# ZpokenWeb3/zk-light-client-implementation

Hardware: AMD Instinct MI355X
Metric: Block_i BFT-finality proofs/sec (100 validators) (higher is better)
Workload: dtype u64

## Files before the change

__graft_entry__.py:

```python
import os
import subprocess
import sys

ROOT = os.path.dirname(os.path.abspath(__file__))
if ROOT not in sys.path:
    sys.path.insert(0, ROOT)


def build() -> None:
    import concurrent.futures
    import importlib
    b = importlib.import_module("zk-light-client-implementation_amd.build")
    pool = concurrent.futures.ThreadPoolExecutor(max_workers=1)
    devsim = pool.submit(b.build_devsim, True)
    b.build(verbose=True)
    mk = os.path.join(ROOT, "oracle", "c", "Makefile")
    if os.path.exists(mk):
        subprocess.check_call(["make", "-s", "-C", os.path.dirname(mk)])
    import zklc_amd
    zklc_amd.load()
    lib_dir = os.path.join(ROOT, "zk-light-client-implementation_amd", "lib")
    subprocess.check_call(["gcc", "-O2", "-Wall", "-Wextra", "-std=c11", "-D_POSIX_C_SOURCE=200809L", "-I", os.path.join(ROOT, "include"),
                           os.path.join(ROOT, "tests", "c_abi", "prove_from_file.c"), "-o", os.path.join(ROOT, "tests", "c_abi", "prove_from_file"),
                           "-L", lib_dir, "-lzklc_mi355", "-Wl,-rpath,$ORIGIN/../../zk-light-client-implementation_amd/lib"])
    b.build_poseidon_gate_dev(True)
    b.build_fri_coeff_dev(True)
    devsim.result()
    pool.shutdown()


def smoke() -> None:
    import json
    import numpy as np
    import zklc_amd
    from oracle import ed25519_ref as ref

    with zklc_amd.Context(0) as ctx:
        j = json.load(open(os.path.join(ROOT, "tests", "golden", "ed25519_near_c1_small.json")))
        msg = bytes.fromhex(j["msg"])
        pks = b"".join(bytes.fromhex(e["validator_tail"])[1:33] for e in j["entries"])
        sigs = b"".join(bytes.fromhex(e["approval"])[2:] for e in j["entries"])
        ok = ctx.ed25519_verify_batch(pks, sigs, msg)
        exp = [int(ref.verify(pks[32 * i:32 * i + 32], sigs[64 * i:64 * i + 64], msg)) for i in range(len(ok))]
        assert ok.tolist() == exp == [1, 1, 1], (ok.tolist(), exp)
        m2 = b"zklc smoke"
        pk2, sg2, exp2 = [], [], []
        for i in range(64):
            sd = ref.synthetic_seed(11, i)
            _, _, pk = ref.keypair(sd)
            s = bytearray(ref.sign(sd, m2))
            if i % 5 == 4:
                s[i % 64] ^= 0x10
            pk2.append(pk)
            sg2.append(bytes(s))
            exp2.append(int(ref.verify(pk, bytes(s), m2)))
        ok2 = ctx.ed25519_verify_batch(b"".join(pk2), b"".join(sg2), m2)
        assert ok2.tolist() == exp2, "GPU Ed25519 batch differs from the oracle"
        assert sum(exp2) == 64 - 12
        from zklc_amd.plonky2 import CircuitBuilder, serialization as S, HASH_GL
        from oracle import plonky2_prover as OP, plonky2_verifier as V
        b = CircuitBuilder()
        x = b.add_virtual_public_input()
        y = b.add_virtual_target()
        z = b.mul(x, y)
        b.split_le(x, 10)
        lo, hi = b.mul_add_u32(x, y, b.constant(77))
        b.register_public_input(lo)
        b.connect(b.sub(b.add(z, b.constant(5)), z), b.constant(5))
        data = b.build()
        wires, pis = data.generate_witness({x: 1000, y: 4000000000})
        prover = data.prover(ctx, HASH_GL)
        raw = prover.prove_bytes(wires, pis)
        common = data.common_data()
        oproof, ovd = OP.prove(common, data.constants, data.sigmas, wires, pis, V.HasherGL)
        assert raw == S.proof_to_bytes(oproof, common, HASH_GL), "GPU plonky2 proof differs from the oracle prover"
        V.verify(json.loads(json.dumps(S.proof_from_bytes(raw, common, HASH_GL))), prover.verifier_data(), common)
        from zklc_amd.plonky2.recursion import RecursionProver
        rp = RecursionProver(ctx, HASH_GL)
        rc, rproof = rp.recursive_proof((common, prover.verifier_data(), raw), None, [7, 8])
        V.verify(json.loads(json.dumps(rproof)), rc.verifier_only, rc.common)
        assert rproof["public_inputs"] == [7, 8]
        bad = bytearray(raw)
        bad[800] ^= 1
        try:
            rp.recursive_proof((common, prover.verifier_data(), bytes(bad)), None, [7, 8])
            raise SystemExit("smoke: a tampered inner proof was accepted by the in-circuit verifier")
        except AssertionError:
            pass
        rp.close()
        prover.close()
    print("smoke OK: Ed25519 batch verify, a plonky2 proof and a recursive proof on cuda:0 match the oracle")


if __name__ == "__main__":
    build()
    if "--smoke" in sys.argv:
        smoke()
```

zk-light-client-implementation_amd/build.py:

```python
import concurrent.futures as cf
import glob
import os
import subprocess
import sys

HERE = os.path.dirname(os.path.abspath(__file__))
CSRC = os.path.join(HERE, "csrc")
BUILD = os.path.join(HERE, "build")
LIBDIR = os.path.join(HERE, "lib")
LIB = os.path.join(LIBDIR, "libzklc_mi355.so")
HIPCC = os.environ.get("HIPCC", "/opt/rocm/bin/hipcc")
FLAGS = ["--offload-arch=gfx950", "-O3", "-std=c++17", "-fPIC", "-fno-gpu-rdc", "-Wall", "-Wno-unused-function"]


def _newest(paths):
    return max((os.path.getmtime(p) for p in paths), default=0.0)


HOST_CXX = os.environ.get("CXX", "g++")
HOST_FLAGS = ["-O3", "-funroll-loops", "-std=c++17", "-fPIC", "-pthread", "-Wall", "-Wno-unused-function", "-Wno-unknown-pragmas"]


def _compile(src, obj, log):
    cmd = ([HIPCC] + FLAGS if src.endswith(".hip") else [HOST_CXX] + HOST_FLAGS) + ["-c", src, "-o", obj]
# ... 20 lines not shown
            jobs.append((s, o))
    if jobs:
        with cf.ThreadPoolExecutor(max_workers=min(len(jobs), os.cpu_count() or 4)) as ex:
            list(ex.map(lambda so: _compile(so[0], so[1], verbose), jobs))
    if jobs or not os.path.exists(LIB) or os.path.getmtime(LIB) < _newest(objs):
        cmd = [HIPCC, "--offload-arch=gfx950", "-shared", "-fPIC", "-pthread", "-o", LIB] + objs
        r = subprocess.run(cmd, capture_output=True, text=True)
        if r.returncode != 0:
            raise RuntimeError("link failed:\n%s\n%s" % (r.stdout, r.stderr))
        if verbose:
            print("[zklc build] linked", LIB, file=sys.stderr)
    return LIB


DEVSIM_DIR = os.path.join(HERE, "..", "tests", "devsim")
DEVSIM_SRC = os.path.join(DEVSIM_DIR, "devsim.hip")
DEVSIM_LIB = os.path.join(DEVSIM_DIR, "libdevsim.so")


def devsim_sources():
    return [DEVSIM_SRC, os.path.abspath(__file__)] + [p for ext in ("*.cuh", "*.h", "*.inc") for p in glob.glob(os.path.join(CSRC, ext))]


def devsim_is_current():
    return os.path.exists(DEVSIM_LIB) and os.path.getmtime(DEVSIM_LIB) >= _newest(devsim_sources())


def build_devsim(verbose=True, force=False):
    if force or not devsim_is_current():
        r = subprocess.run([HIPCC] + FLAGS + ["-shared", DEVSIM_SRC, "-o", DEVSIM_LIB], capture_output=True, text=True)
        if r.returncode != 0:
            raise RuntimeError("hipcc failed for %s:\n%s\n%s" % (DEVSIM_SRC, r.stdout, r.stderr))
        if verbose:
            print("[zklc build] built", DEVSIM_LIB, file=sys.stderr)
    return DEVSIM_LIB


PGD_DIR = os.path.join(HERE, "..", "tests", "poseidon_gate_dev")
PGD_SRC = os.path.join(PGD_DIR, "poseidon_gate_dev.hip")
PGD_LIB = os.path.join(PGD_DIR, "libposeidon_gate_dev.so")


def poseidon_gate_dev_is_current():
    deps = [PGD_SRC, os.path.abspath(__file__)] + [p for ext in ("*.cuh", "*.h", "*.inc") for p in glob.glob(os.path.join(CSRC, ext))]
    return os.path.exists(PGD_LIB) and os.path.getmtime(PGD_LIB) >= _newest(deps)


def build_poseidon_gate_dev(verbose=True, force=False):
    if force or not poseidon_gate_dev_is_current():
        r = subprocess.run([HIPCC] + FLAGS + ["-Wno-inline-asm", "-shared", PGD_SRC, "-o", PGD_LIB], capture_output=True, text=True)
        if r.returncode != 0:
            raise RuntimeError("hipcc failed for %s:\n%s\n%s" % (PGD_SRC, r.stdout, r.stderr))
        if verbose:
            print("[zklc build] built", PGD_LIB, file=sys.stderr)
    return PGD_LIB


FCD_DIR = os.path.join(HERE, "..", "tests", "fri_coeff_dev")
FCD_SRC = os.path.join(FCD_DIR, "fri_coeff_dev.hip")
FCD_CASES = os.path.join(FCD_DIR, "fri_coeff_dev_cases.cpp")
FCD_LIB = os.path.join(FCD_DIR, "libfri_coeff_dev.so")


def fri_coeff_dev_is_current():
    deps = [FCD_SRC, FCD_CASES, os.path.join(HERE, "..", "tests", "fri_coeff_host", "fri_coeff_cases.h"), os.path.abspath(__file__)]
    deps += [p for ext in ("*.cuh", "*.h", "*.inc") for p in glob.glob(os.path.join(CSRC, ext))]
    return os.path.exists(FCD_LIB) and os.path.getmtime(FCD_LIB) >= _newest(deps)


def build_fri_coeff_dev(verbose=True, force=False):
    if force or not fri_coeff_dev_is_current():
        obj, kobj = os.path.join(FCD_DIR, "fri_coeff_dev_cases.o"), os.path.join(FCD_DIR, "fri_coeff_dev.o")
        for cmd in ([HOST_CXX, "-O2", "-std=c++17", "-fPIC", "-Wall", "-Wno-unused-function", "-Wno-unknown-pragmas", "-c", FCD_CASES, "-o", obj],
                    [HIPCC] + FLAGS + ["-c", FCD_SRC, "-o", kobj],
                    [HIPCC, "--offload-arch=gfx950", "-shared", "-fPIC", "-o", FCD_LIB, kobj, obj]):
            r = subprocess.run(cmd, capture_output=True, text=True)
            if r.returncode != 0:
                raise RuntimeError("%s failed for %s:\n%s\n%s" % (cmd[0], FCD_DIR, r.stdout[-4000:], r.stderr[-4000:]))
        if verbose:
            print("[zklc build] built", FCD_LIB, file=sys.stderr)
    return FCD_LIB


if __name__ == "__main__":
    build(force="--force" in sys.argv)
    build_devsim(force="--force" in sys.argv)
    build_poseidon_gate_dev(force="--force" in sys.argv)
    build_fri_coeff_dev(force="--force" in sys.argv)
```

zk-light-client-implementation_amd/csrc/plonky2_prover.hip:

```cpp
#include <algorithm>
#include <chrono>
#include <stdio.h>
#include <stdlib.h>
#include <new>
#include <vector>
#include <string.h>
#include "plonky2_gates.cuh"
#include "plonky2_host.h"
#include "plonky2_perm_terms.cuh"
#include "plonky2_fri_combine.cuh"
#include "zklc_internal.h"

#define P2_THREADS 256

struct p2_challenges {
    u64 beta[P2_MAX_CH], gamma[P2_MAX_CH], alpha[P2_MAX_CH];
};

__global__ void p2_pow_table_kernel(u64 *out, u64 base, u64 n) {
    u64 i = (u64)blockIdx.x * blockDim.x + threadIdx.x;
    if (i < n) out[i] = gl_pow(base, i);
}

__global__ void p2_scale_by_powers_kernel(u64 *data, u64 base, u64 n) {
    u64 j = (u64)blockIdx.x * blockDim.x + threadIdx.x;
    if (j >= n) return;
    u64 *p = data + (size_t)blockIdx.y * n + j;
    *p = gl_mul(*p, gl_pow(base, j));
}

#define P2_SCALE_PER_LANE 8
__global__ void __launch_bounds__(256) p2_scale_by_powers_strided_kernel(u64 *data, u64 base, u64 step, u64 n) {
    const u64 j0 = (u64)blockIdx.x * (256 * P2_SCALE_PER_LANE) + threadIdx.x;
    if (j0 >= n) return;
    u64 *p = data + (size_t)blockIdx.y * n;
    u64 v[P2_SCALE_PER_LANE];
#pragma unroll
    for (int q = 0; q < P2_SCALE_PER_LANE; q++) v[q] = j0 + 256 * q < n ? p[j0 + 256 * q] : 0;
    u64 pw = gl_pow(base, j0);
#pragma unroll
    for (int q = 0; q < P2_SCALE_PER_LANE; q++) {
        if (j0 + 256 * q < n) p[j0 + 256 * q] = gl_mul(v[q], pw);
        if (q + 1 < P2_SCALE_PER_LANE) pw = gl_mul(pw, step);
    }
}

__global__ void p2_ext_powers_kernel(gl2 *out, gl2 z, u64 n) {
    u64 j = (u64)blockIdx.x * blockDim.x + threadIdx.x;
    if (j < n) out[j] = gl2_pow(z, j);
}

__global__ void p2_ext_pow_limbs_kernel(u32 *out, gl2 z, u32 n) {
    u32 j = blockIdx.x * blockDim.x + threadIdx.x;
    if (j >= n) return;
    gl2 v = gl2_pow(z, j);
    gl_limbs22(v.a, out + 12 * (size_t)j);
    gl_limbs22(v.b, out + 12 * (size_t)j + 6);
}

template <bool LEAN>
__global__ void __launch_bounds__(P2_THREADS)
p2_chunk_products_kernel(const u64 *__restrict__ wires, const u64 *__restrict__ sigmas, const u64 *__restrict__ subgroup,
                         const u64 *__restrict__ k_is, u32 n, u32 routed, u32 qdf, u32 nchunks, u64 beta, u64 gamma,
                         u64 *__restrict__ rp) {
    u32 i = blockIdx.x * blockDim.x + threadIdx.x;
    if (i >= n) return;
    u64 x = subgroup[i];
    u64 nums[16], dens[16];
    for (u32 k = 0; k < nchunks; k++) {
        u64 np = 1, dp = 1;
        u32 end = (k + 1) * qdf < routed ? (k + 1) * qdf : routed;
        if constexpr (LEAN) {
            const u64 bx = gl_mul(beta, x);
            for (u32 j = k * qdf; j < end; j += P2_PERM_CHUNK) {
                const u32 cnt = end - j < P2_PERM_CHUNK ? end - j : P2_PERM_CHUNK;
                u64 wv[P2_PERM_CHUNK], sv[P2_PERM_CHUNK], kv[P2_PERM_CHUNK], n8, d8;
#pragma unroll
                for (u32 q = 0; q < P2_PERM_CHUNK; q++) {
                    const u32 jq = q < cnt ? j + q : j;
                    wv[q] = wires[(size_t)jq * n + i];
                    sv[q] = sigmas[(size_t)jq * n + i];
                    kv[q] = k_is[jq];
                }
                p2_perm_chunk_terms(wv, sv, kv, cnt, beta, bx, gamma, n8, d8);
                if (j == k * qdf) {
                    np = n8;
                    dp = d8;
                } else {
                    np = gl_mul(np, n8);
                    dp = gl_mul(dp, d8);
                }
            }
        } else {
// ... 485 lines not shown
                    tw[(size_t)(first + j - base) * 64 + lane] = w[j];
                    trp[(size_t)(first + j - base) * 64 + lane] = rp[j];
                }
        }
        __syncthreads();
        const u32 ntop = base;
        const bool more = ntop > plan.lo;
        const u32 nbase = !more ? plan.lo : (ntop - plan.lo > P2_AMT_COLS ? ntop - P2_AMT_COLS : plan.lo);
        if (more) {
            const u32 first = nbase + wave * per_wave;
#pragma unroll
            for (u32 j = 0; j < per_wave; j++) {
                const u32 col = first + j < ntop ? first + j : ntop - 1;
                wn[j] = W[(size_t)col * N];
            }
        }
        if (OPS[0]) p2_amt_consume<0>(acc, comb, OPS[0], L0[0], base, top, tw, trp, lane, apow, (int)a.nch, k0);
        if (OPS[1]) p2_amt_consume<1>(acc, comb, OPS[1], L0[1], base, top, tw, trp, lane, apow, (int)a.nch, k0);
        __syncthreads();
        if (!more) break;
        top = ntop;
        base = nbase;
    }
    u64 sum[P2_MAX_CH];
#pragma unroll
    for (int c = 0; c < P2_MAX_CH; c++) sum[c] = 0;
    p2_vars sv;
    sv.consts = a.cs;
    sv.stride = N;
    sv.p = p;
    sv.nsel = a.nsel;
#pragma unroll
    for (int s = 0; s < 2; s++) {
        if (GI[s] == 0xFFFFFFFFu) continue;
        const p2_gate g = a.gates[GI[s]];
        const u64 f = p2_filter(GI[s], g.group_start, g.group_end, sv.sel(g.selector_index), a.nsel > 1);
#pragma unroll
        for (int c = 0; c < P2_MAX_CH; c++)
            if (c < (int)a.nch) sum[c] = gl_add(sum[c], gl_mul(f, gl_acc3_reduce(acc[s][c])));
    }
    u64 *part = tw;
#pragma unroll
    for (int c = 0; c < P2_MAX_CH; c++) part[((size_t)wave * P2_MAX_CH + c) * 64 + lane] = sum[c];
    __syncthreads();
    if (wave == 0) {
        const u64 pi = __brevll((u64)p) >> (64 - a.lde_bits);
        const u64 zi = a.zh_inv[(u32)pi & ((1u << a.rate_bits) - 1)];
#pragma unroll
        for (int c = 0; c < P2_MAX_CH; c++)
            if (c < (int)a.nch) {
                u64 t = sum[c];
                for (u32 w = 1; w < P2_AMT_WAVES; w++) t = gl_add(t, part[((size_t)w * P2_MAX_CH + c) * 64 + lane]);
                u64 *o = a.out + (size_t)c * N + p;
                *o = gl_add(*o, gl_mul(t, zi));
            }
    }
}
static bool p2_amt_make_plan(const p2_gate *gates, const p2_gate_list &list, p2_amt_plan &plan) {
    if (list.n < 2 || list.n > 2 * P2_AMT_WAVES) return false;
    u32 load[P2_AMT_WAVES] = {0, 0, 0, 0}, used[P2_AMT_WAVES] = {0, 0, 0, 0};
    for (int w = 0; w < P2_AMT_WAVES; w++) plan.slot[w][0] = plan.slot[w][1] = 0xFFFFFFFFu;
    plan.lo = 0xFFFFFFFFu;
    plan.hi = 0;
    bool taken[P2_GATE_LIST_MAX] = {};
    for (u32 r = 0; r < list.n; r++) {
        u32 best = 0xFFFFFFFFu;
        for (u32 t = 0; t < list.n; t++)
            if (!taken[t] && (best == 0xFFFFFFFFu || gates[list.idx[t]].p[1] > gates[list.idx[best]].p[1])) best = t;
        taken[best] = true;
        const p2_gate &g = gates[list.idx[best]];
        const u32 ops = g.p[1], l0 = (g.p[0] + 3) * ops;
        if (ops == 0 || 24 * ops >= 480) return false;
        u32 w = 0xFFFFFFFFu;
        for (u32 k = 0; k < P2_AMT_WAVES; k++)
            if (used[k] < 2 && (w == 0xFFFFFFFFu || load[k] < load[w])) w = k;
        plan.slot[w][used[w]++] = best;
        load[w] += ops;
        plan.lo = l0 < plan.lo ? l0 : plan.lo;
        plan.hi = l0 + 18 * ops > plan.hi ? l0 + 18 * ops : plan.hi;
    }
    return plan.hi > plan.lo;
}

typedef void (*p2_gate_kernel_fn)(p2_quotient_args, p2_gate_list);
static p2_gate_kernel_fn p2_gate_kernel_of(u32 type) {
    static const char *pg = getenv("ZKLC_P2_POSEIDON_GATE");
    if (type == P2_POSEIDON && (!pg || !pg[0] || !strcmp(pg, "stmt"))) return p2_quotient_poseidon_stmt_kernel;
    if (type == P2_POSEIDON && !strcmp(pg, "loose")) return p2_quotient_gate_kernel<P2_POSEIDON_LOOSE>;
    if (type == P2_POSEIDON && pg && !strncmp(pg, "lazy", 4)) {
        return pg[4] == '1' ? p2_quotient_gate_kernel<P2_POSEIDON_LAZY + 1> : p2_quotient_gate_kernel<P2_POSEIDON_LAZY>;
    }
    switch (type) {
#define P2_CASE(T) case T: return p2_quotient_gate_kernel<T>;
        P2_CASE(P2_CONSTANT) P2_CASE(P2_PUBLIC_INPUT) P2_CASE(P2_ARITHMETIC) P2_CASE(P2_ARITHMETIC_EXT) P2_CASE(P2_MUL_EXT)
        P2_CASE(P2_BASE_SUM) P2_CASE(P2_POSEIDON) P2_CASE(P2_POSEIDON_MDS) P2_CASE(P2_RANDOM_ACCESS) P2_CASE(P2_REDUCING)
        P2_CASE(P2_REDUCING_EXT) P2_CASE(P2_EXPONENTIATION) P2_CASE(P2_COSET_INTERPOLATION) P2_CASE(P2_U32_ARITHMETIC)
        P2_CASE(P2_U32_ADD_MANY) P2_CASE(P2_U32_SUBTRACTION) P2_CASE(P2_U32_RANGE_CHECK) P2_CASE(P2_COMPARISON)
        P2_CASE(P2_U32_INTERLEAVE) P2_CASE(P2_UNINTERLEAVE_TO_U32) P2_CASE(P2_UNINTERLEAVE_TO_B32)
#undef P2_CASE
        default: return nullptr;
    }
}

#define P2_FQ_MAX_WAVES 8
#define P2_FQ_MAX_JOBS 40
#define P2_JOB_BASE 0xFFFFu
struct p2_fused_plan {
    u32 nwaves;
    u32 njobs[P2_FQ_MAX_WAVES];
    uint16_t jobs[P2_FQ_MAX_WAVES][P2_FQ_MAX_JOBS];
};

__global__ void __launch_bounds__(64 * P2_FQ_MAX_WAVES) p2_quotient_fused_kernel(p2_quotient_args a, p2_fused_plan plan) {
    extern __shared__ u64 p2_tile[];
    const size_t N = (size_t)1 << a.lde_bits;
    const u32 lane = threadIdx.x & 63;
    const u32 wave = __builtin_amdgcn_readfirstlane(threadIdx.x >> 6);
    const size_t p = (size_t)blockIdx.x * 64 + lane;
    const u32 ncols = a.num_constants + a.num_wires;
    {
        u32 j = wave;
        for (; j + 7 * plan.nwaves < ncols; j += 8 * plan.nwaves) {
            u64 t[8];
#pragma unroll
            for (int q = 0; q < 8; q++) {
                u32 jj = j + q * plan.nwaves;
                const u64 *src = jj < a.num_constants ? a.cs + (size_t)jj * N : a.wires + (size_t)(jj - a.num_constants) * N;
                t[q] = src[p];
            }
#pragma unroll
            for (int q = 0; q < 8; q++) p2_tile[(size_t)(j + q * plan.nwaves) * 64 + lane] = t[q];
        }
        for (; j < ncols; j += plan.nwaves) {
            const u64 *src = j < a.num_constants ? a.cs + (size_t)j * N : a.wires + (size_t)(j - a.num_constants) * N;
            p2_tile[(size_t)j * 64 + lane] = src[p];
        }
    }
    __syncthreads();
    p2_vars_lds v;
    v.consts = (p2_lds_u64 *)p2_tile;
    v.wires = v.consts + (size_t)a.num_constants * 64;
    v.lane = lane;
    v.nsel = a.nsel;
    for (int k = 0; k < 4; k++) v.pih[k] = a.pih[k];
    u64 sum[P2_MAX_CH] = {0, 0};
    p2_consumer out;
    out.nch = a.nch;
    for (int c = 0; c < P2_MAX_CH; c++) out.apow[c] = (gl_ktab *)a.apow[c];
    const u32 njobs = plan.njobs[wave];
    for (u32 jb = 0; jb < njobs; jb++) {
        const u32 g = plan.jobs[wave][jb];
        if (g == P2_JOB_BASE) {
            u64 i = __brevll((u64)p) >> (64 - a.lde_bits);
            u64 x = a.xs[p], l0 = a.l0[p];
            u64 i_next = (i + (1ULL << a.rate_bits)) & (N - 1);
            size_t p_next = (size_t)(__brevll(i_next) >> (64 - a.lde_bits));
            out.reset(0);
            for (u32 c = 0; c < a.nch; c++) out.emit(gl_mul(l0, gl_sub(a.zs[(size_t)c * N + p], 1)));
            const u32 nchunks = a.npp + 1;
            for (u32 c = 0; c < a.nch; c++) {
                u64 beta = a.ch.beta[c], gamma = a.ch.gamma[c];
                u64 prev = a.zs[(size_t)c * N + p];
                for (u32 k = 0; k < nchunks; k++) {
                    u64 np = 1, dp = 1;
                    u32 end = (k + 1) * a.qdf < a.routed ? (k + 1) * a.qdf : a.routed;
                    for (u32 j = k * a.qdf; j < end; j++) {
// ... 772 lines not shown
    hipStream_t st = zklc_pick_stream(ctx, stream);
    const u32 n = c->n, N = c->N, nch = P.num_challenges, npp = P.num_partial_products;
    const int hasher = (int)P.hasher;
    double t0 = p2_now_ms(), t_prev = t0;
    auto lap = [&](int slot) {
        double t = p2_now_ms();
        c->timings[slot] = t - t_prev;
        t_prev = t;
    };
    c->last_challenges.clear();
    p2_pin_reset(c);

    u64 pih[4];
    zklc_host_poseidon_hash_no_pad(public_inputs, P.num_public_inputs, pih);
    zklc_challenger ch;
    ch.observe_hash(c->digest, hasher);
    ch.observe_many(pih, 4);

    std::vector<uint8_t> wires_cap, zs_cap, quot_cap;
    P2_RC(zklc_gl_intt_copy_dev(ctx, st, d_wires, c->wires.coeffs, P.degree_bits, P.num_wires));
    P2_RC(p2_commit_coeffs(c, st, c->wires, wires_cap));
    p2_observe_cap(ch, wires_cap, hasher);
    p2_challenges chal = {};
    for (u32 k = 0; k < nch; k++) chal.beta[k] = ch.challenge();
    for (u32 k = 0; k < nch; k++) chal.gamma[k] = ch.challenge();
    lap(0);

    u32 nblocks = (n + P2_SCAN_BLOCK - 1) / P2_SCAN_BLOCK;
    P2_PIN(c, grand, u64, P2_MAX_CH);
    for (u32 k = 0; k < P2_MAX_CH; k++) grand[k] = 1;
    for (u32 k = 0; k < nch; k++) {
        hipLaunchKernelGGL(zklc_lean_arith() ? p2_chunk_products_kernel<true> : p2_chunk_products_kernel<false>,
                           dim3((n + P2_THREADS - 1) / P2_THREADS), dim3(P2_THREADS), 0, st, d_wires,
                           (const u64 *)c->d_sigma_vals, (const u64 *)c->d_subgroup, (const u64 *)c->d_kis, n, P.num_routed_wires,
                           P.quotient_degree_factor, c->nchunks, chal.beta[k], chal.gamma[k], c->d_rp);
        hipLaunchKernelGGL(p2_scan_local_kernel, dim3(nblocks), dim3(P2_THREADS), 0, st, (const u64 *)(c->d_rp + (size_t)npp * n),
                           c->d_excl, c->d_totals, n);
        hipLaunchKernelGGL(p2_scan_totals_kernel, dim3(1), dim3(P2_THREADS), 0, st, c->d_totals, nblocks, c->d_grand);
        hipLaunchKernelGGL(p2_z_apply_kernel, dim3((n + P2_THREADS - 1) / P2_THREADS), dim3(P2_THREADS), 0, st, (const u64 *)c->d_excl,
                           (const u64 *)c->d_totals, (const u64 *)c->d_rp, n, npp, c->zs.coeffs + (size_t)k * n,
                           c->zs.coeffs + (size_t)(nch + k * npp) * n);
        ZKLC_HIP(ctx, hipGetLastError());
        ZKLC_HIP(ctx, zklc_readback_async(&grand[k], c->d_grand, 8, st));
    }
    P2_RC(p2_commit_values(c, st, c->zs, zs_cap));
    for (u32 k = 0; k < nch; k++)
        if (grand[k] != 1) {
            ctx->last_err = "plonky2: the witness violates the copy constraints (permutation product != 1)";
            return ZKLC_ERR_INVALID_ARG;
        }
    p2_observe_cap(ch, zs_cap, hasher);
    for (u32 k = 0; k < nch; k++) chal.alpha[k] = ch.challenge();
    lap(1);

    {
        p2_quotient_args a = {};
        p2_quotient_static_args(c, a);
        for (int k = 0; k < 4; k++) a.pih[k] = pih[k];
        a.ch = chal;
        {
            u32 n_pow = nch + nch * (npp + 1) + P.num_gate_constraints + 1;
            P2_PIN(c, tab, u32, (size_t)nch * n_pow * 6);
            for (u32 k = 0; k < nch; k++) {
                u64 v = 1;
                for (u32 i = 0; i < n_pow; i++) {
                    u32 *t6 = &tab[((size_t)k * n_pow + i) * 6];
                    const u64 v2 = h_mul(v, 1ULL << 32);
                    t6[0] = (u32)(v & 0x3FFFFF), t6[1] = (u32)((v >> 22) & 0x3FFFFF), t6[2] = (u32)(v >> 44);
                    t6[3] = (u32)(v2 & 0x3FFFFF), t6[4] = (u32)((v2 >> 22) & 0x3FFFFF), t6[5] = (u32)(v2 >> 44);
                    v = h_mul(v, chal.alpha[k]);
                }
            }
            ZKLC_HIP(ctx, hipMemcpyAsync(c->d_apow, tab, (size_t)nch * n_pow * 6 * 4, hipMemcpyHostToDevice, st));
            for (u32 k = 0; k < nch; k++) a.apow[k] = c->d_apow + (size_t)k * n_pow * 6;
            for (u32 k = nch; k < P2_MAX_CH; k++) a.apow[k] = c->d_apow;
        }
        if (c->plan.nwaves) {
            hipLaunchKernelGGL(p2_quotient_fused_kernel, dim3(N / 64), dim3(64 * c->plan.nwaves), c->fused_lds, st, a, c->plan);
        } else {
            hipLaunchKernelGGL(zklc_lean_arith() ? p2_quotient_base_kernel<true> : p2_quotient_base_kernel<false>,
                               dim3((N + P2_THREADS - 1) / P2_THREADS), dim3(P2_THREADS), 0, st, a);
            static const bool one_per_launch = getenv("ZKLC_P2_GATE_LAUNCH") && !strcmp(getenv("ZKLC_P2_GATE_LAUNCH"), "single");
            std::vector<bool> done(P.num_gates, false);
            for (u32 g = 0; g < P.num_gates; g++) {
                p2_gate_kernel_fn fn = p2_gate_kernel_of(c->gates[g].type);
                if (!fn || done[g]) continue;
                p2_gate_list list = {};
                for (u32 h = g; h < P.num_gates && list.n < (one_per_launch ? 1u : (u32)P2_GATE_LIST_MAX); h++)
                    if (!done[h] && c->gates[h].type == c->gates[g].type) {
                        list.idx[list.n++] = h;
                        done[h] = true;
                    }
                static const bool am_multi = getenv("ZKLC_P2_ADDMANY") && !strcmp(getenv("ZKLC_P2_ADDMANY"), "multi");
                static const bool am_pergate = getenv("ZKLC_P2_ADDMANY") && !strcmp(getenv("ZKLC_P2_ADDMANY"), "pergate");
                static const bool am_check = getenv("ZKLC_P2_ADDMANY") && !strcmp(getenv("ZKLC_P2_ADDMANY"), "check");
                if (am_check && c->gates[g].type == P2_U32_ADD_MANY && N >= 64) {
                    p2_amt_plan plan;
                    if (p2_amt_make_plan(c->gates.data(), list, plan)) {
                        u64 *s1 = nullptr, *s2 = nullptr;
                        const size_t words = (size_t)nch * N;
                        ZKLC_HIP(ctx, hipMalloc(&s1, words * 8));
                        ZKLC_HIP(ctx, hipMalloc(&s2, words * 8));
                        ZKLC_HIP(ctx, hipMemsetAsync(s1, 0, words * 8, st));
                        ZKLC_HIP(ctx, hipMemsetAsync(s2, 0, words * 8, st));
                        p2_quotient_args b1 = a, b2 = a;
                        b1.out = s1;
                        b2.out = s2;
                        hipLaunchKernelGGL(fn, dim3((N + P2_THREADS - 1) / P2_THREADS), dim3(P2_THREADS), 0, st, b1, list);
                        hipLaunchKernelGGL(p2_quotient_addmany_tile_kernel, dim3(N / 64), dim3(64 * P2_AMT_WAVES), 0, st, b2, list, plan);
                        std::vector<u64> h1(words), h2(words);
                        ZKLC_HIP(ctx, hipMemcpyAsync(h1.data(), s1, words * 8, hipMemcpyDeviceToHost, st));
                        ZKLC_HIP(ctx, hipMemcpyAsync(h2.data(), s2, words * 8, hipMemcpyDeviceToHost, st));
                        ZKLC_HIP(ctx, zklc_stream_wait(st));
                        size_t bad = 0;
                        for (size_t i = 0; i < words; i++) bad += h1[i] % GL_P != h2[i] % GL_P;
                        fprintf(stderr, "[zklc] addmany check: %u variants, limb columns [%u, %u): %zu of %zu values differ\n", list.n, plan.lo,
                                plan.hi, bad, words);
                        (void)hipFree(s1);
                        (void)hipFree(s2);
                    }
                }
                if (c->gates[g].type == P2_U32_ADD_MANY && !am_multi && !am_pergate && !am_check && N >= 64) {
                    p2_amt_plan plan;
                    if (p2_amt_make_plan(c->gates.data(), list, plan)) {
                        hipLaunchKernelGGL(p2_quotient_addmany_tile_kernel, dim3(N / 64), dim3(64 * P2_AMT_WAVES), 0, st, a, list, plan);
                        continue;
                    }
                }
                if (am_multi && c->gates[g].type == P2_U32_ADD_MANY && list.n >= 2 && list.n <= P2_AM_MAX)
                    fn = p2_quotient_addmany_multi_kernel;
                hipLaunchKernelGGL(fn, dim3((N + P2_THREADS - 1) / P2_THREADS), dim3(P2_THREADS), 0, st, a, list);
            }
        }
        ZKLC_HIP(ctx, hipGetLastError());
        P2_RC(zklc_gl_ntt_dev(ctx, st, c->d_qv, c->lde_bits, nch, ZKLC_NTT_INVERSE | ZKLC_NTT_IN_BITREV, 0));
        if (zklc_lean_arith()) {
            const u64 gi = h_inv(GL_GENERATOR);
            hipLaunchKernelGGL(p2_scale_by_powers_strided_kernel, dim3((N + 256 * P2_SCALE_PER_LANE - 1) / (256 * P2_SCALE_PER_LANE), nch),
                               dim3(256), 0, st, c->d_qv, gi, h_pow(gi, 256), (u64)N);
        } else {
            hipLaunchKernelGGL(p2_scale_by_powers_kernel, dim3((N + 255) / 256, nch), dim3(256), 0, st, c->d_qv, h_inv(GL_GENERATOR), (u64)N);
        }
        ZKLC_HIP(ctx, hipGetLastError());
        P2_RC(p2_commit_coeffs(c, st, c->quot, quot_cap));
    }
    p2_observe_cap(ch, quot_cap, hasher);
    gl2 zeta;
    zeta.a = ch.challenge();
    zeta.b = ch.challenge();
    lap(2);

    const u32 w0 = c->cs.width, w1 = c->wires.width, w2 = c->zs.width, w3 = c->quot.width;
    const u32 n_open = w0 + w1 + w2 + w3 + nch;
    P2_PIN(c, open, gl2, n_open);
    {
        hipLaunchKernelGGL(p2_ext_powers_kernel, dim3((n + 255) / 256), dim3(256), 0, st, c->d_zpow, zeta, (u64)n);
        const p2_batch *bs[4] = {&c->cs, &c->wires, &c->zs, &c->quot};
        u32 off = 0;
        for (int k = 0; k < 4; k++) {
            hipLaunchKernelGGL(p2_eval_at_ext_kernel, dim3(bs[k]->width, P2_EVAL_SPLIT), dim3(P2_THREADS), 0, st,
                               (const u64 *)bs[k]->coeffs, n, (const gl2 *)c->d_zpow, (const u64 *)nullptr,
                               c->d_open_partial + (size_t)off * P2_EVAL_SPLIT);
            off += bs[k]->width;
        }
        hipLaunchKernelGGL(p2_eval_at_ext_kernel, dim3(nch, P2_EVAL_SPLIT), dim3(P2_THREADS), 0, st, (const u64 *)c->zs.coeffs, n,
                           (const gl2 *)c->d_zpow, (const u64 *)c->d_subgroup, c->d_open_partial + (size_t)off * P2_EVAL_SPLIT);
// ... 304 lines not shown
```

Measured before the change: 0.2288.

## Fuse u32 arithmetic, subtraction and range-check gates into one shared limb-walk quotient kernel

Adds a quotient kernel that evaluates up to three u32-family gates (arithmetic, subtraction, range check) in one launch. It walks their overlapping limb wire columns once, sharing wire loads and range products across the gates, and accumulates per-gate alpha-weighted sums that are filtered at the end. The aim is to remove repeated global reads of the same limb columns and separate per-gate launches. It is on by default, and a check mode compares it against the per-gate kernels. The risk is the complex column-to-constraint mapping and reduced occupancy from the per-thread accumulators.

New measurement: 0.2305 (median of 6 runs). Within noise of the previous version (+0.8%).

```diff
diff --git a/__graft_entry__.py b/__graft_entry__.py
--- a/__graft_entry__.py
+++ b/__graft_entry__.py
@@ -25,6 +25,7 @@
                            "-L", lib_dir, "-lzklc_mi355", "-Wl,-rpath,$ORIGIN/../../zk-light-client-implementation_amd/lib"])
     b.build_poseidon_gate_dev(True)
     b.build_fri_coeff_dev(True)
+    b.build_u32_walk_dev(True)
     devsim.result()
     pool.shutdown()
 
diff --git a/zk-light-client-implementation_amd/build.py b/zk-light-client-implementation_amd/build.py
--- a/zk-light-client-implementation_amd/build.py
+++ b/zk-light-client-implementation_amd/build.py
@@ -126,8 +126,29 @@
     return FCD_LIB
 
 
+UWD_DIR = os.path.join(HERE, "..", "tests", "u32_walk_dev")
+UWD_SRC = os.path.join(UWD_DIR, "u32_walk_dev.hip")
+UWD_LIB = os.path.join(UWD_DIR, "libu32_walk_dev.so")
+
+
+def u32_walk_dev_is_current():
+    deps = [UWD_SRC, os.path.abspath(__file__)] + [p for ext in ("*.cuh", "*.h", "*.inc") for p in glob.glob(os.path.join(CSRC, ext))]
+    return os.path.exists(UWD_LIB) and os.path.getmtime(UWD_LIB) >= _newest(deps)
+
+
+def build_u32_walk_dev(verbose=True, force=False):
+    if force or not u32_walk_dev_is_current():
+        r = subprocess.run([HIPCC] + FLAGS + ["-Wno-inline-asm", "-shared", UWD_SRC, "-o", UWD_LIB], capture_output=True, text=True)
+        if r.returncode != 0:
+            raise RuntimeError("hipcc failed for %s:\n%s\n%s" % (UWD_SRC, r.stdout, r.stderr))
+        if verbose:
+            print("[zklc build] built", UWD_LIB, file=sys.stderr)
+    return UWD_LIB
+
+
 if __name__ == "__main__":
     build(force="--force" in sys.argv)
     build_devsim(force="--force" in sys.argv)
     build_poseidon_gate_dev(force="--force" in sys.argv)
     build_fri_coeff_dev(force="--force" in sys.argv)
+    build_u32_walk_dev(force="--force" in sys.argv)
diff --git a/zk-light-client-implementation_amd/csrc/plonky2_prover.hip b/zk-light-client-implementation_amd/csrc/plonky2_prover.hip
--- a/zk-light-client-implementation_amd/csrc/plonky2_prover.hip
+++ b/zk-light-client-implementation_amd/csrc/plonky2_prover.hip
@@ -9,6 +9,7 @@
 #include "plonky2_host.h"
 #include "plonky2_perm_terms.cuh"
 #include "plonky2_fri_combine.cuh"
+#include "plonky2_u32_walk.cuh"
 #include "zklc_internal.h"
 
 #define P2_THREADS 256
@@ -660,6 +661,14 @@
     return plan.hi > plan.lo;
 }
 
+template <int NCH>
+__global__ void __launch_bounds__(64, 3) p2_quotient_u32_walk_kernel(p2_quotient_args a, p2_u32w_plan plan) {
+    const size_t p = (size_t)blockIdx.x * 64 + threadIdx.x;
+    p2_u32w_point<NCH>(a, plan, p);
+}
+static_assert(P2_MAX_CH == 2, "p2_quotient_u32_walk_kernel is instantiated for one and two challenges");
+#define P2_U32W_DEFAULT 1
+
 typedef void (*p2_gate_kernel_fn)(p2_quotient_args, p2_gate_list);
 static p2_gate_kernel_fn p2_gate_kernel_of(u32 type) {
     static const char *pg = getenv("ZKLC_P2_POSEIDON_GATE");
@@ -1598,6 +1607,47 @@
                                dim3((N + P2_THREADS - 1) / P2_THREADS), dim3(P2_THREADS), 0, st, a);
             static const bool one_per_launch = getenv("ZKLC_P2_GATE_LAUNCH") && !strcmp(getenv("ZKLC_P2_GATE_LAUNCH"), "single");
             std::vector<bool> done(P.num_gates, false);
+            {
+                static const char *uw = getenv("ZKLC_P2_U32WALK");
+                static const bool uw_set = uw && uw[0], uw_check = uw_set && !strcmp(uw, "check"), uw_walk = uw_set && !strcmp(uw, "walk");
+                static const bool uw_on = uw_check || uw_walk || (!uw_set && P2_U32W_DEFAULT);
+                p2_u32w_plan wplan;
+                auto walk_kernel = nch == 1 ? p2_quotient_u32_walk_kernel<1> : p2_quotient_u32_walk_kernel<2>;
+                if (uw_on && p2_u32w_make_plan(c->gates.data(), P.num_gates, P.num_wires, (u64)N, wplan)) {
+                    if (uw_check) {
+                        u64 *s1 = nullptr, *s2 = nullptr;
+                        const size_t words = (size_t)nch * N;
+                        ZKLC_HIP(ctx, hipMalloc(&s1, words * 8));
+                        ZKLC_HIP(ctx, hipMalloc(&s2, words * 8));
+                        ZKLC_HIP(ctx, hipMemsetAsync(s1, 0, words * 8, st));
+                        ZKLC_HIP(ctx, hipMemsetAsync(s2, 0, words * 8, st));
+                        p2_quotient_args b1 = a, b2 = a;
+                        b1.out = s1;
+                        b2.out = s2;
+                        for (u32 k = 0; k < wplan.n; k++) {
+                            p2_gate_list one = {};
+                            one.n = 1;
+                            one.idx[0] = wplan.r[k].gate;
+                            hipLaunchKernelGGL(p2_gate_kernel_of(wplan.r[k].type), dim3((N + P2_THREADS - 1) / P2_THREADS), dim3(P2_THREADS), 0, st,
+                                               b1, one);
+                        }
+                        hipLaunchKernelGGL(walk_kernel, dim3(N / 64), dim3(64), 0, st, b2, wplan);
+                        std::vector<u64> h1(words), h2(words);
+                        ZKLC_HIP(ctx, zklc_readback_async(h1.data(), s1, words * 8, st));
+                        ZKLC_HIP(ctx, zklc_readback_async(h2.data(), s2, words * 8, st));
+                        ZKLC_HIP(ctx, zklc_stream_wait(st));
+                        size_t bad = 0;
+                        for (size_t i = 0; i < words; i++) bad += h1[i] % GL_P != h2[i] % GL_P;
+                        fprintf(stderr, "[zklc] u32 walk check: %u gates, limb columns [%u, %u): %zu of %zu values differ\n", wplan.n, wplan.lo,
+                                wplan.hi, bad, words);
+                        (void)hipFree(s1);
+                        (void)hipFree(s2);
+                    } else {
+                        hipLaunchKernelGGL(walk_kernel, dim3(N / 64), dim3(64), 0, st, a, wplan);
+                        for (u32 k = 0; k < wplan.n; k++) done[wplan.r[k].gate] = true;
+                    }
+                }
+            }
             for (u32 g = 0; g < P.num_gates; g++) {
                 p2_gate_kernel_fn fn = p2_gate_kernel_of(c->gates[g].type);
                 if (!fn || done[g]) continue;
diff --git a/zk-light-client-implementation_amd/csrc/plonky2_u32_walk.cuh b/zk-light-client-implementation_amd/csrc/plonky2_u32_walk.cuh
--- /dev/null
+++ b/zk-light-client-implementation_amd/csrc/plonky2_u32_walk.cuh
@@ -0,0 +1,234 @@
+#pragma once
+#include "plonky2_gates.cuh"
+
+#define P2_U32W_MAX 3
+#define P2_U32W_NONE 0xFFFFFFFFu
+struct p2_u32w_region {
+    u32 gate;
+    u32 type;
+    u32 l0;
+    u32 ops;
+    u32 map;
+};
+struct p2_u32w_plan {
+    u32 n;
+    u32 lo, hi;
+    p2_u32w_region r[P2_U32W_MAX];
+};
+#if defined(__HIPCC__)
+#define P2_U32W_BOTH __host__ __device__ __forceinline__
+#else
+#define P2_U32W_BOTH static inline
+#endif
+#define P2_U32W_MAP(lg, cpo, kl0, ksum, up, two) ((u32)(lg) | (u32)(cpo) << 3 | (u32)(kl0) << 9 | (u32)(ksum) << 15 | (u32)(up) << 21 | (u32)(two) << 22)
+P2_U32W_BOTH u32 p2_u32w_lg(u32 map) { return map & 7; }
+P2_U32W_BOTH u32 p2_u32w_cpo(u32 map) { return (map >> 3) & 63; }
+P2_U32W_BOTH u32 p2_u32w_kl0(u32 map) { return (map >> 9) & 63; }
+P2_U32W_BOTH u32 p2_u32w_ksum(u32 map) { return (map >> 15) & 63; }
+P2_U32W_BOTH bool p2_u32w_up(u32 map) { return (map >> 21) & 1; }
+P2_U32W_BOTH bool p2_u32w_two_sums(u32 map) { return (map >> 22) & 1; }
+P2_U32W_BOTH u32 p2_u32w_limbs(const p2_u32w_region &r) { return r.ops << p2_u32w_lg(r.map); }
+P2_U32W_BOTH u32 p2_u32w_end(const p2_u32w_region &r) { return r.l0 + p2_u32w_limbs(r); }
+P2_U32W_BOTH u32 p2_u32w_num_constraints(const p2_u32w_region &r) { return p2_u32w_cpo(r.map) * r.ops; }
+P2_U32W_BOTH u32 p2_u32w_limb_constraint(u32 map, u32 i, u32 l) {
+    return p2_u32w_cpo(map) * i + (p2_u32w_up(map) ? p2_u32w_kl0(map) + l : p2_u32w_kl0(map) - l);
+}
+
+static inline bool p2_u32w_region_of(const p2_gate &g, u32 index, p2_u32w_region &r) {
+    r.gate = index;
+    r.type = g.type;
+    r.ops = g.p[0];
+    switch (g.type) {
+        case P2_U32_ARITHMETIC: r.l0 = 6 * r.ops, r.map = P2_U32W_MAP(5, 36, 33, 34, 0, 1); return true;
+        case P2_U32_SUBTRACTION: r.l0 = 5 * r.ops, r.map = P2_U32W_MAP(4, 19, 16, 17, 0, 0); return true;
+        case P2_U32_RANGE_CHECK: r.l0 = r.ops, r.map = P2_U32W_MAP(4, 17, 1, 0, 1, 0); return true;
+        default: return false;
+    }
+}
+static inline bool p2_u32w_make_plan(const p2_gate *gates, u32 num_gates, u32 num_wires, u64 lde_points, p2_u32w_plan &plan) {
+    plan.n = 0;
+    plan.lo = 0xFFFFFFFFu;
+    plan.hi = 0;
+    for (u32 k = 0; k < P2_U32W_MAX; k++) plan.r[k] = p2_u32w_region{P2_U32W_NONE, 0, 0, 0, 0};
+    if (lde_points < 64) return false;
+    for (u32 g = 0; g < num_gates; g++) {
+        p2_u32w_region r;
+        if (!p2_u32w_region_of(gates[g], g, r)) continue;
+        if (r.ops == 0 || r.ops > 480 || p2_u32w_num_constraints(r) > 480 || p2_u32w_end(r) > num_wires) return false;
+        u32 pos = plan.n;
+        while (pos > 0 && p2_u32w_limbs(plan.r[pos - 1]) < p2_u32w_limbs(r)) pos--;
+        if (pos >= P2_U32W_MAX) continue;
+        for (u32 k = (plan.n < P2_U32W_MAX ? plan.n : P2_U32W_MAX - 1); k > pos; k--) plan.r[k] = plan.r[k - 1];
+        plan.r[pos] = r;
+        if (plan.n < P2_U32W_MAX) plan.n++;
+    }
+    if (plan.n < 2) return false;
+    for (u32 k = 0; k < plan.n; k++) {
+        plan.lo = plan.r[k].l0 < plan.lo ? plan.r[k].l0 : plan.lo;
+        plan.hi = p2_u32w_end(plan.r[k]) > plan.hi ? p2_u32w_end(plan.r[k]) : plan.hi;
+    }
+    return plan.hi > plan.lo;
+}
+
+template <int R, int NCH, class V>
+ZKLC_D void p2_u32w_routed(gl_acc3 (&acc)[P2_U32W_MAX][P2_MAX_CH], const V &pv, const p2_u32w_region &r, gl_ktab *const (&apow)[P2_MAX_CH],
+                           u32 k0) {
+    auto emit = [&](u32 krel, u64 val) __attribute__((always_inline)) {
+#pragma unroll
+        for (int c = 0; c < NCH; c++) gl_acc3_mul(acc[R][c], val, apow[c] + 6 * (size_t)(k0 + krel));
+    };
+#if defined(__HIPCC__)
+#pragma unroll 1
+#endif
+    for (u32 i = 0; i < r.ops; i++) {
+        const u32 kb = p2_u32w_cpo(r.map) * i;
+        if (r.type == P2_U32_ARITHMETIC) {
+            u64 w[6];
+            p2_load<6>(pv, 6 * i, w);
+            const u64 m0 = w[0], m1 = w[1], add = w[2], lo = w[3], hi = w[4], inv = w[5];
+            const u64 computed = gl_add(gl_mul(m0, m1), add);
+            const u64 diff = gl_sub(0xFFFFFFFFULL, hi);
+            const u64 hi_not_max = gl_sub(gl_mul(inv, diff), 1);
+            emit(kb, gl_mul(hi_not_max, lo));
+            emit(kb + 1, gl_sub(gl_add(gl_mul(hi, 1ULL << 32), lo), computed));
+            emit(kb + 34, gl_neg(lo));
+            emit(kb + 35, gl_neg(hi));
+        } else if (r.type == P2_U32_SUBTRACTION) {
+            u64 w[5];
+            p2_load<5>(pv, 5 * i, w);
+            const u64 x = w[0], y = w[1], bin = w[2], res = w[3], bout = w[4];
+            const u64 initial = gl_sub(gl_sub(x, y), bin);
+            emit(kb, gl_sub(res, gl_add(initial, gl_mul(bout, 1ULL << 32))));
+            emit(kb + 17, gl_neg(res));
+            emit(kb + 18, gl_mul(bout, gl_sub(1, bout)));
+        } else {
+            emit(kb, gl_neg(pv.w(i)));
+        }
+    }
+}
+
+template <int R, int NCH>
+ZKLC_D void p2_u32w_step4(gl_acc3 (&acc)[P2_U32W_MAX][P2_MAX_CH], u64 &cb, const p2_u32w_region &r, int top, const u64 (&w)[4],
+                          const u64 (&rp)[4], gl_ktab *const (&apow)[P2_MAX_CH], u32 k0) {
+    u32 map = r.map;
+#if defined(__HIP_DEVICE_COMPILE__)
+    asm volatile("" : "+s"(map));
+#endif
+    const u32 lg = p2_u32w_lg(map);
+    const int l0 = (int)r.l0, end = l0 + (int)(r.ops << lg);
+    if (top <= l0 || top - 4 >= end) return;
+    const u32 lmask = (1u << lg) - 1;
+    u32 k[4], je = 4, ks = 0;
+    bool in[4];
+#pragma unroll
+    for (int j = 0; j < 4; j++) {
+        const int col = top - 1 - j;
+        in[j] = col < end && col >= l0;
+        const u32 rel = in[j] ? (u32)(col - l0) : 0u, i = rel >> lg, l = rel & lmask;
+        k[j] = k0 + p2_u32w_limb_constraint(map, i, l);
+        if (in[j] && (l == 0 || (l == 16 && p2_u32w_two_sums(map)))) je = (u32)j, ks = k0 + p2_u32w_cpo(map) * i + p2_u32w_ksum(map) + (l ? 1 : 0);
+    }
+#pragma unroll
+    for (int c = 0; c < NCH; c++) {
+        if (c) P2_SCHED_FENCE();
+#pragma unroll
+        for (int j = 0; j < 4; j++) gl_acc3_mul(acc[R][c], in[j] ? rp[j] : 0, apow[c] + 6 * (size_t)k[j]);
+    }
+    u64 s = 0;
+#pragma unroll
+    for (int j = 0; j < 4; j++) {
+        cb = in[j] ? p2_horner4(cb, w[j]) : cb;
+        const bool done = je == (u32)j;
+        s = done ? cb : s;
+        cb = done ? 0 : cb;
+    }
+    if (je < 4) {
+        s = gl_canonical(s);
+#pragma unroll
+        for (int c = 0; c < NCH; c++) gl_acc3_mul(acc[R][c], s, apow[c] + 6 * (size_t)ks);
+    }
+}
+
+#define P2_U32W_AHEAD 1
+template <int NCH, class V>
+ZKLC_D void p2_u32w_walk(gl_acc3 (&acc)[P2_U32W_MAX][P2_MAX_CH], const V &pv, const p2_u32w_plan &plan, gl_ktab *const (&apow)[P2_MAX_CH],
+                         u32 k0) {
+#pragma unroll
+    for (int s = 0; s < P2_U32W_MAX; s++)
+#pragma unroll
+        for (int c = 0; c < P2_MAX_CH; c++) acc[s][c].c0 = acc[s][c].c1 = acc[s][c].c2 = 0;
+    p2_u32w_routed<0, NCH>(acc, pv, plan.r[0], apow, k0);
+    p2_u32w_routed<1, NCH>(acc, pv, plan.r[1], apow, k0);
+    if (P2_U32W_MAX > 2 && plan.n > 2) p2_u32w_routed<2, NCH>(acc, pv, plan.r[2], apow, k0);
+
+    const int lo = (int)plan.lo;
+    int top = (int)plan.hi;
+    u64 wn[P2_U32W_AHEAD][4];
+#pragma unroll
+    for (int b = 0; b < P2_U32W_AHEAD; b++)
+#pragma unroll
+        for (int j = 0; j < 4; j++) {
+            const int col = top - 4 * b - 1 - j;
+            wn[b][j] = pv.w((u32)(col > lo ? col : lo));
+        }
+    u64 cb0 = 0, cb1 = 0, cb2 = 0;
+#if defined(__HIPCC__)
+#pragma unroll 1
+#endif
+    for (; top > lo; top -= 4) {
+        u64 w[4], rp[4];
+#pragma unroll
+        for (int j = 0; j < 4; j++) w[j] = wn[0][j];
+#pragma unroll
+        for (int b = 0; b + 1 < P2_U32W_AHEAD; b++)
+#pragma unroll
+            for (int j = 0; j < 4; j++) wn[b][j] = wn[b + 1][j];
+#pragma unroll
+        for (int j = 0; j < 4; j++) {
+            const int col = top - 4 * P2_U32W_AHEAD - 1 - j;
+            wn[P2_U32W_AHEAD - 1][j] = pv.w((u32)(col > lo ? col : lo));
+        }
+        p2_range_products4<4>(w, rp);
+        p2_u32w_step4<0, NCH>(acc, cb0, plan.r[0], top, w, rp, apow, k0);
+        p2_u32w_step4<1, NCH>(acc, cb1, plan.r[1], top, w, rp, apow, k0);
+        if (P2_U32W_MAX > 2 && plan.n > 2) p2_u32w_step4<2, NCH>(acc, cb2, plan.r[2], top, w, rp, apow, k0);
+    }
+}
+
+#if defined(__HIPCC__)
+template <int NCH, class A>
+ZKLC_D void p2_u32w_point(const A &a, const p2_u32w_plan &plan, size_t p) {
+    const size_t N = (size_t)1 << a.lde_bits;
+    const u32 k0 = a.nch + a.nch * (a.npp + 1);
+    gl_acc3 acc[P2_U32W_MAX][P2_MAX_CH];
+    gl_ktab *apow[P2_MAX_CH];
+#pragma unroll
+    for (int c = 0; c < P2_MAX_CH; c++) apow[c] = (gl_ktab *)a.apow[c];
+    p2_vars pv;
+    pv.wires = a.wires;
+    pv.consts = a.cs;
+    pv.stride = N;
+    pv.p = p;
+    pv.nsel = a.nsel;
+    p2_u32w_walk<NCH>(acc, pv, plan, apow, k0);
+    u64 sum[P2_MAX_CH];
+#pragma unroll
+    for (int c = 0; c < P2_MAX_CH; c++) sum[c] = 0;
+#pragma unroll
+    for (int s = 0; s < P2_U32W_MAX; s++) {
+        if (s >= (int)plan.n) continue;
+        const u32 gi = plan.r[s].gate;
+        const p2_gate g = a.gates[gi];
+        const u64 f = p2_filter(gi, g.group_start, g.group_end, pv.sel(g.selector_index), a.nsel > 1);
+#pragma unroll
+        for (int c = 0; c < NCH; c++) sum[c] = gl_add(sum[c], gl_mul(f, gl_acc3_reduce(acc[s][c])));
+    }
+    const u64 pi = __brevll((u64)p) >> (64 - a.lde_bits);
+    const u64 zi = a.zh_inv[(u32)pi & ((1u << a.rate_bits) - 1)];
+#pragma unroll
+    for (int c = 0; c < NCH; c++) {
+        u64 *o = a.out + (size_t)c * N + p;
+        *o = gl_add(*o, gl_mul(sum[c], zi));
+    }
+}
+#endif
```
